# JokerJohn/Cloud_Map_Evaluation

Hardware: AMD Instinct MI355X
Metric: Mpts/sec full metric suite (CD+MME+AWD) on 50M-pt pair (higher is better)
Workload: dtype f64

## Files before the change

cloud_map_evaluation_amd/csrc/me_nn.hip:

```cpp
#include <cmath>
#include <cstdlib>

#include "me_internal.hpp"
#include "me_stat.hpp"

#ifndef ME_NN_DBG
#define ME_NN_DBG 0
#endif

namespace me {

__device__ __forceinline__ double vmin_f64(double a, double b) {
    double r;
    asm("v_min_f64 %0, %1, %2" : "=v"(r) : "v"(a), "v"(b));
    return r;
}

__device__ __forceinline__ float fminf_raw(float a, float b) {
    float r;
    asm("v_min_f32_e32 %0, %1, %2" : "=v"(r) : "v"(a), "v"(b));
    return r;
}

__device__ __forceinline__ double vmax_f64(double a, double b) {
    double r;
    asm("v_max_f64 %0, %1, %2" : "=v"(r) : "v"(a), "v"(b));
    return r;
}

__device__ __forceinline__ double box_lower_bound(const float *__restrict__ b, double qx, double qy, double qz) {
    const double dx = fmax(fmax((double) b[0] - qx, qx - (double) b[3]), 0.0);
    const double dy = fmax(fmax((double) b[1] - qy, qy - (double) b[4]), 0.0);
    const double dz = fmax(fmax((double) b[2] - qz, qz - (double) b[5]), 0.0);
    return (dx * dx + dy * dy) + dz * dz;
}

__device__ __forceinline__ double box_lower_bound_cov(const float *__restrict__ b, double qx, double qy, double qz, int axis, double clo,
                                                      double chi) {
    double d[3];
    d[0] = fmax(fmax((double) b[0] - qx, qx - (double) b[3]), 0.0);
    d[1] = fmax(fmax((double) b[1] - qy, qy - (double) b[4]), 0.0);
    d[2] = fmax(fmax((double) b[2] - qz, qz - (double) b[5]), 0.0);
    const double qa = axis == 0 ? qx : (axis == 1 ? qy : qz);
    const double lo = axis == 0 ? (double) b[0] : (axis == 1 ? (double) b[1] : (double) b[2]);
    const double hi = axis == 0 ? (double) b[3] : (axis == 1 ? (double) b[4] : (double) b[5]);
    if (qa >= clo && qa < chi) {
        const double up = hi >= chi ? fmax(lo, chi) - qa : INFINITY;
        const double dn = lo < clo ? qa - fmin(hi, clo) : INFINITY;
        const double da = fmin(up, dn);
        if (axis == 0) d[0] = da;
        else if (axis == 1) d[1] = da;
        else d[2] = da;
    }
    return (d[0] * d[0] + d[1] * d[1]) + d[2] * d[2];
}

__device__ __forceinline__ double box_upper_bound(const float *__restrict__ b, double qx, double qy, double qz) {
    const double dx = fmax(fabs(qx - (double) b[0]), fabs(qx - (double) b[3]));
    const double dy = fmax(fabs(qy - (double) b[1]), fabs(qy - (double) b[4]));
    const double dz = fmax(fabs(qz - (double) b[2]), fabs(qz - (double) b[5]));
    return (dx * dx + dy * dy) + dz * dz;
}

template <bool FROM_LIST>
__global__ void __launch_bounds__(256) __attribute__((amdgpu_waves_per_eu(8, 8)))
k_nn_grid(const SPoint *__restrict__ qsp, long long q_begin, long long q_end, const SPoint *__restrict__ rsp, long long nr,
          GridView g,
          FrameView fr, SlabView slab, double *__restrict__ d2_out, int *__restrict__ idx_out,
          unsigned int *__restrict__ list, unsigned int *__restrict__ list_count, unsigned int xcd_chunk,
          const unsigned int *__restrict__ in_list, const unsigned int *__restrict__ in_count, unsigned char *__restrict__ flag_out) {
    const int lane = threadIdx.x & 63;
    const unsigned int vb = FROM_LIST ? blockIdx.x : xcd_virtual_block(blockIdx.x, gridDim.x, xcd_chunk);
    const int cell_bits = kMortonBits - g.shift;
    const int cell_lim = 1 << cell_bits;
    const double cell_h = ldexp(fr.fine_h, g.shift);
    __shared__ float4 s_tile[4][64];
    static_assert(sizeof(s_tile[0]) >= kGroupRowsEnt * 4, "the row masks and keys of the round's table alias the wave's tile");
    __shared__ int2 s_tab[4][kGroupTab + 1];
    const unsigned int n_in = FROM_LIST ? *in_count : 0u;
  for (unsigned int pos = vb * blockDim.x + threadIdx.x;; pos += gridDim.x * blockDim.x) {
    unsigned int qoff;
    bool active;
    if (FROM_LIST) {
        if (!__ballot(pos < n_in)) break;
        active = pos < n_in;
        qoff = active ? in_list[pos] : 0u;
    } else {
        qoff = pos;
        active = q_begin + (long long) qoff < q_end;
    }

    double qx = 0, qy = 0, qz = 0;
    int mcx = 0, mcy = 0, mcz = 0;
    bool in_grid = false;
    if (active) {
        unsigned int qo = qoff;
        asm volatile("" : "+v"(qo));
        const SPoint q = qsp[q_begin + (long long) qo];
        qx = q.x;
        qy = q.y;
        qz = q.z;
        if (!FROM_LIST && !slab_owned(slab, qx, qy, qz)) {
            d2_out[q_begin + (long long) qo] = -1.0;
            idx_out[q_begin + (long long) qo] = -1;
            active = false;
        }
    }
    if (active) {
        const double fx = fine_coord(qx, fr.ox, fr.fine_h), fy = fine_coord(qy, fr.oy, fr.fine_h),
                     fz = fine_coord(qz, fr.oz, fr.fine_h);
        const double lim = 2097151.0;
        in_grid = fx >= 0.0 && fy >= 0.0 && fz >= 0.0 && fx <= lim && fy <= lim && fz <= lim;
        if (in_grid) {
            mcx = (int) ((unsigned int) fx >> g.shift);
            mcy = (int) ((unsigned int) fy >> g.shift);
            mcz = (int) ((unsigned int) fz >> g.shift);
        }
    }
    float b1 = INFINITY, b2 = INFINITY, b3 = INFINITY;
    int j1 = -1, j2 = -1;
    bool done = !active || !in_grid;

    float ax = 0, ay = 0, az = 0;
    bool in_round = false;
    const float rank_tol = (float) (1e-3 * cell_h * cell_h);
#if ME_TUNE_NN_SGPR_MASKS
    auto note = [&](float m, int j) {
        unsigned long long lt1, lt2;
        asm("v_cmp_lt_f32_e64 %0, %1, %2" : "=s"(lt1) : "v"(m), "v"(b1));
        asm("v_cmp_lt_f32_e64 %0, %1, %2" : "=s"(lt2) : "v"(m), "v"(b2));
        b3 = __builtin_amdgcn_fmed3f(b2, b3, m);
        b2 = __builtin_amdgcn_fmed3f(b1, b2, m);
        int jn;
        asm("v_cndmask_b32_e64 %0, %1, %2, %3" : "=v"(jn) : "v"(j2), "v"(j), "s"(lt2));
        asm("v_cndmask_b32_e64 %0, %1, %2, %3" : "=v"(j2) : "v"(jn), "v"(j1), "s"(lt1));
        asm("v_min_f32_e32 %0, %1, %2" : "=v"(b1) : "v"(b1), "v"(m));
        asm("v_cndmask_b32_e64 %0, %1, %2, %3" : "=v"(j1) : "v"(j1), "v"(j), "s"(lt1));
    };
#else
    auto note = [&](float m, int j) {
        const bool lt1 = m < b1, lt2 = m < b2;
        b3 = __builtin_amdgcn_fmed3f(b2, b3, m);
        b2 = __builtin_amdgcn_fmed3f(b1, b2, m);
        const int jn = lt2 ? j : j2;
        j2 = lt1 ? j1 : jn;
        b1 = lt1 ? m : b1;
        j1 = lt1 ? j : j1;
    };
#endif
    float4 *tile = s_tile[threadIdx.x >> 6];
    double ox = 0, oy = 0, oz = 0;
    auto rank = [&](int j) {
        const float4 c = tile[j];
        return fmaf(c.x, ax, fmaf(c.y, ay, fmaf(c.z, az, c.w)));
    };
    auto min3 = [](float a, float b, float c) { return __builtin_amdgcn_fmed3f(-INFINITY, a, __builtin_amdgcn_fmed3f(-INFINITY, b, c)); };
    double px64 = 0, py64 = 0, pz64 = 0;
    auto load_chunk = [&](int base, int n) {
        if (lane < n && ME_NN_DBG != 2) {
            const SPoint p = rsp[(ME_NN_DBG == 5) ? ((base + lane) & 4095) : (base + lane)];
            px64 = p.x;
            py64 = p.y;
            pz64 = p.z;
        }
    };
    auto stage_chunk = [&](int n) {
        const int n4 = (n + 3) & ~3;
        if (lane < n4 && ME_NN_DBG != 2) {
            float4 rec = make_float4(0.0f, 0.0f, 0.0f, INFINITY);
            if (lane < n) {
                const double px = px64 - ox, py = py64 - oy, pz = pz64 - oz;
                rec = make_float4((float) px, (float) py, (float) pz, (float) fma(pz, pz, fma(py, py, px * px)));
            }
            tile[lane] = rec;
        }
        __builtin_amdgcn_fence(__ATOMIC_ACQ_REL, "wavefront");
        __builtin_amdgcn_wave_barrier();
    };
    auto rank_chunk = [&](int base, int n) {
        const int n4 = (n + 3) & ~3;
        if (in_round && ME_NN_DBG != 1 && ME_NN_DBG != 2) {
            int j = 0;
#if ME_NN_DBG == 4
            float acc = 0.0f;
            for (; j < n4; ++j) acc += rank(j);
            if (acc == 12345.0f) note(acc, base);
            j = n4;
#endif
            for (; j + 8 <= n4; j += 8) {
                const float m0 = min3(rank(j), rank(j + 1), rank(j + 2));
                const float m1 = min3(rank(j + 3), rank(j + 4), rank(j + 5));
                note(min3(m0, m1, fminf_raw(rank(j + 6), rank(j + 7))), base + j);
            }
            if (j < n4) note(min3(rank(j), rank(j + 1), fminf_raw(rank(j + 2), rank(j + 3))), base + j);
        }
        __builtin_amdgcn_fence(__ATOMIC_ACQ_REL, "wavefront");
        __builtin_amdgcn_wave_barrier();
    };
    int2 *tab = s_tab[threadIdx.x >> 6];
    while (__ballot(!done)) {
        GroupBox bx;
        int nk = 0;
        const bool in = wave_group_table<1, true, kGroupR, false, true>(!done, mcx, mcy, mcz, g, cell_lim, lane, tab, bx, &nk,
                                                  reinterpret_cast<unsigned int *>(tile));
        ox = uniform_f64(fr.ox + (double) bx.x0 * cell_h);
        oy = uniform_f64(fr.oy + (double) bx.y0 * cell_h);
        oz = uniform_f64(fr.oz + (double) bx.z0 * cell_h);
        if (in) {
            unsigned int qo = qoff;
            asm volatile("" : "+v"(qo));
            const SPoint q = qsp[q_begin + (long long) qo];
            ax = (float) (-2.0 * (q.x - ox));
            ay = (float) (-2.0 * (q.y - oy));
            az = (float) (-2.0 * (q.z - oz));
        }
        in_round = in;
        int it_blk = -64, it_pos = 0, it_end = 0;
        unsigned long long it_m = 0;
        auto next_chunk = [&](int &cbase, int &cn) -> bool {
            if (it_pos >= it_end) {
                while (!it_m) {
                    it_blk += 64;
                    if (it_blk >= nk) return false;
                    const int t = it_blk + lane;
                    const int cnt = (t < nk) ? tab[t].y : 0;
                    it_m = __ballot(cnt > 0);
                }
                const int sidx = __ffsll((long long) it_m) - 1;
                it_m &= it_m - 1;
                const int2 run = tab[it_blk + sidx];
                it_pos = __builtin_amdgcn_readfirstlane(run.x);
                it_end = it_pos + __builtin_amdgcn_readfirstlane(run.y);
                while (it_m) {
                    const int s2 = __ffsll((long long) it_m) - 1;
                    const int2 nx = tab[it_blk + s2];
                    if (__builtin_amdgcn_readfirstlane(nx.x) != it_end) break;
                    it_end += __builtin_amdgcn_readfirstlane(nx.y);
                    it_m &= it_m - 1;
                }
            }
            cbase = it_pos;
            cn = min(64, it_end - it_pos);
            it_pos += cn;
            return true;
        };
        int cb = 0, cn = 0;
        bool have = next_chunk(cb, cn);
        if (have) load_chunk(cb, cn);
        while (have) {
            stage_chunk(cn);
            int nb2 = 0, nn2 = 0;
            const bool nhave = next_chunk(nb2, nn2);
            if (nhave) load_chunk(nb2, nn2);
            rank_chunk(cb, cn);
            have = nhave;
            cb = nb2;
            cn = nn2;
        }
        if (in) done = true;
        __builtin_amdgcn_wave_barrier();
    }

    bool unresolved = false;
    if (active) {
        unresolved = true;
        {
            unsigned int qo = qoff;
            asm volatile("" : "+v"(qo));
            const SPoint q = qsp[q_begin + (long long) qo];
            qx = q.x;
            qy = q.y;
            qz = q.z;
        }
        double best_x = INFINITY;
        long long best_i = 0x7fffffffffffffffLL;
        auto exact_group = [&](int jg) {
            if (jg < 0 || ME_NN_DBG == 3) return;
#pragma unroll
            for (int t = 0; t < 8; ++t) {
                const long long pos = (long long) jg + t;
                if (pos < nr) {
                    const SPoint p = rsp[pos];
                    const double e = dist2_exact(qx, qy, qz, p.x, p.y, p.z);
                    if (e < best_x || (e == best_x && p.idx < best_i)) {
                        best_x = e;
                        best_i = p.idx;
                    }
                }
            }
        };
        exact_group(j1);
        if (!(b2 - b1 > rank_tol)) exact_group(j2);
        const bool ranking_safe = b3 - b1 > rank_tol;
        if (in_grid && j1 >= 0 && ranking_safe) {
            const double lox = fr.ox + (double) (mcx - 1) * cell_h, hix = fr.ox + (double) (mcx + 2) * cell_h;
            const double loy = fr.oy + (double) (mcy - 1) * cell_h, hiy = fr.oy + (double) (mcy + 2) * cell_h;
            const double loz = fr.oz + (double) (mcz - 1) * cell_h, hiz = fr.oz + (double) (mcz + 2) * cell_h;
            double gmin = fmin(fmin(qx - lox, hix - qx), fmin(fmin(qy - loy, hiy - qy), fmin(qz - loz, hiz - qz)));
            gmin *= (1.0 - 1e-9);
            unresolved = !(gmin > 0.0 && best_x < gmin * gmin);
        }
        unsigned int qo = qoff;
        asm volatile("" : "+v"(qo));
        d2_out[q_begin + (long long) qo] = best_x;
        idx_out[q_begin + (long long) qo] = (j1 >= 0) ? (int) best_i : -1;
    }
    if (ME_NN_DBG) unresolved = false;
    if (!FROM_LIST && flag_out) {
        if (q_begin + (long long) qoff < q_end) flag_out[qoff] = unresolved ? 1 : 0;
    } else {
        const unsigned long long um = __ballot(unresolved);
        if (um) {
            unsigned int base = 0;
            if (lane == 0) base = atomicAdd(list_count, (unsigned int) __popcll(um));
            base = (unsigned int) readlane_i((int) base, 0);
            if (unresolved) list[base + (unsigned int) __popcll(um & ((1ULL << lane) - 1ULL))] = qoff;
        }
    }
    if (!FROM_LIST) break;
    __builtin_amdgcn_wave_barrier();
  }
}

#ifdef ME_AB
#include "me_nn_kernels_ab.inc"
#endif

__device__ __forceinline__ double octet_min(double v) {
    v = fmin(v, octet_partner_d<0>(v));
    v = fmin(v, octet_partner_d<1>(v));
    v = fmin(v, octet_partner_d<2>(v));
    return v;
}

constexpr int kNn1Block = 64;
constexpr int kNn1Waves = 5;
template <bool COV, bool DBG>
__global__ void __launch_bounds__(kNn1Block) __attribute__((amdgpu_waves_per_eu(kNn1Waves, 8)))
k_nn1(const SPoint *__restrict__ qsp, long long q_begin, long long q_end, const SPoint *__restrict__ rsp, long long nr,
      OctView oct, double *__restrict__ d2_out, int *__restrict__ idx_out, const unsigned int *__restrict__ list,
      const unsigned int *__restrict__ list_count, int use_bound, unsigned long long *__restrict__ dbg,
      unsigned int *__restrict__ far_list, unsigned int *__restrict__ far_count, int far_cap, unsigned int *__restrict__ work,
      const double *__restrict__ cov, int cov_axis) {
    __shared__ long long s_off[kMaxLevels];
    extern __shared__ unsigned int s_dyn[];
    if (threadIdx.x < kMaxLevels) s_off[threadIdx.x] = oct.off[threadIdx.x];
    __syncthreads();
    const int L = oct.n_levels - 1;
    const int lv = oct.n_levels + 1;
    const ONode *__restrict__ nodes = oct.nodes;
    const long long n_items = list ? (long long) *list_count : (q_end - q_begin);
    const int sub = threadIdx.x & 7;
    const unsigned long long t_wave0 = DBG ? wall_clock64() : 0ULL;
    unsigned long long w_open = 0, w_scan = 0, w_pts = 0;
    unsigned int w_max = 0;
    static_assert(kNn1Block == 64, "one wavefront per block: the group counter is drawn by lane 0 of the block");
    for (long long g = blockIdx.x;;) {
        const long long t = g * 8 + (threadIdx.x >> 3);
        const bool alive = t < n_items;
        if (!__ballot(alive)) break;
        {
            unsigned int nx = 0;
            if (threadIdx.x == 0) nx = atomicAdd(work, 1u);
            g = (long long) gridDim.x + (long long) (unsigned int) __builtin_amdgcn_readfirstlane((int) nx);
        }
        const long long i = q_begin + (alive ? (list ? (long long) list[t] : t) : 0);
        const SPoint q = qsp[i];
        const double qx = q.x, qy = q.y, qz = q.z;
        double clo = INFINITY, chi = -INFINITY;
        if (COV && alive) {
            clo = cov[2 * (i - q_begin)];
            chi = cov[2 * (i - q_begin) + 1];
        }
        unsigned int n_open = 0, n_scan = 0;
        unsigned long long n_pts = 0;
        double best = INFINITY;
        long long best_i = 0x7fffffffffffffffLL;
        if (list && alive) {
            best = d2_out[i];
            const int bi = idx_out[i];
            if (bi >= 0) best_i = bi;
        } else if (use_bound && alive) {
            best = d2_out[i];
        }
        double lb = best;
        long long li = best_i;
        double bound = best;
        auto scan_points = [&](bool go, long long jb, long long je) {
            if (!go) jb = je = 0;
            if (DBG) {
                n_scan += go ? 1u : 0u;
                n_pts += (unsigned long long) (je - jb);
            } else {
                n_open += go ? 1u : 0u;
            }
            for (long long j = jb + sub; __ballot(j < je); j += 16) {
                const long long j1 = j + 8;
                const long long last = je > 0 ? je - 1 : 0;
                const SPoint p0 = rsp[j < je ? j : last];
                const SPoint p1 = rsp[j1 < je ? j1 : last];
                const double d0 = dist2_exact(qx, qy, qz, p0.x, p0.y, p0.z);
                const double d1 = dist2_exact(qx, qy, qz, p1.x, p1.y, p1.z);
                if (j < je && (d0 < lb || (d0 == lb && p0.idx < li))) {
                    lb = d0;
                    li = p0.idx;
                }
                if (j1 < je && (d1 < lb || (d1 == lb && p1.idx < li))) {
                    lb = d1;
                    li = p1.idx;
                }
            }
            int m = __float_as_int(__double2float_ru(lb));
            m = min(m, octet_partner_i<0>(m));
            m = min(m, octet_partner_i<1>(m));
            m = min(m, octet_partner_i<2>(m));
            if (go) bound = fmin(bound, (double) __int_as_float(m));
        };
        bool far_flag = false;
        if (L == 0) {
            scan_points(alive, 0, nr);
        } else {
            float *c_lb = reinterpret_cast<float *>(s_dyn) + (threadIdx.x >> 3) * lv * 8;
            unsigned int *c_beg = s_dyn + (kNn1Block / 8) * lv * 8 + (threadIdx.x >> 3) * lv * 9;
            unsigned long long taken_lo = 0, taken_hi = 0;
            bool walking = alive;
            int l = L;
            struct Fetched {
                float4 a, bb;
                unsigned int nxt;
            };
            auto open_load = [&](bool go, int lev, long long cb) {
                if (!go) {
                    cb = 0;
                    lev = 1;
                }
                const long long at = s_off[lev - 1] + cb + sub;
                const float4 *__restrict__ g = reinterpret_cast<const float4 *>(nodes + at);
                Fetched f;
                f.a = g[0];
                f.bb = g[1];
                f.nxt = nodes[at + 1].begin;
                return f;
            };
            auto open_finish = [&](bool go, int lev, long long cb, long long ce, const Fetched &ft) {
                if (!go) {
                    cb = ce = 0;
                    lev = 1;
                }
                const int cnt = (int) (ce - cb);
                n_open += go ? 1u : 0u;
                const float f[6] = {ft.a.x, ft.a.y, ft.a.z, ft.a.w, ft.bb.x, ft.bb.y};
                const bool mine = go && sub < cnt;
                const double ub = octet_min(mine ? box_upper_bound(f, qx, qy, qz) : INFINITY);
                const double lbd = COV ? box_lower_bound_cov(f, qx, qy, qz, cov_axis, clo, chi) : box_lower_bound(f, qx, qy, qz);
                if (go) {
                    bound = fmin(bound, ub);
                    c_lb[lev * 8 + sub] = mine ? __double2float_rd(lbd) : INFINITY;
                    c_beg[lev * 9 + sub] = __float_as_uint(ft.bb.z);
// ... 387 lines not shown
    const long long i = (long long) blockIdx.x * blockDim.x + threadIdx.x;
    bool un = false;
    if (i < n) {
        const double d = d2[i];
        if (d >= 0.0) {
            const SPoint q = qsp[i];
            const double f = slab_face_distance(slab, q.x, q.y, q.z);
            un = !(d < f * f);
        }
    }
    const unsigned long long um = __ballot(un);
    if (um) {
        const int lane = threadIdx.x & 63;
        unsigned int base = 0;
        if (lane == 0) base = atomicAdd(count, (unsigned int) __popcll(um));
        base = (unsigned int) readlane_i((int) base, 0);
        if (un) list[base + (unsigned int) __popcll(um & ((1ULL << lane) - 1ULL))] = (unsigned int) i;
    }
}

__global__ void k_nn_export_xyz(const SPoint *__restrict__ qsp, const unsigned int *__restrict__ list, long long m,
                                double *__restrict__ xyz, const double *__restrict__ d2s, double *__restrict__ d2) {
    const long long t = (long long) blockIdx.x * blockDim.x + threadIdx.x;
    if (t >= m) return;
    const SPoint q = qsp[list[t]];
    if (d2) d2[t] = d2s[list[t]];
    xyz[3 * t] = q.x;
    xyz[3 * t + 1] = q.y;
    xyz[3 * t + 2] = q.z;
}

__global__ void k_points_to_sp(const double *__restrict__ xyz, long long m, SPoint *__restrict__ sp) {
    const long long t = (long long) blockIdx.x * blockDim.x + threadIdx.x;
    if (t >= m) return;
    SPoint p;
    p.x = xyz[3 * t];
    p.y = xyz[3 * t + 1];
    p.z = xyz[3 * t + 2];
    p.idx = t;
    sp[t] = p;
}

__global__ void k_fill_f64(double *p, long long n, double v) {
    const long long t = (long long) blockIdx.x * blockDim.x + threadIdx.x;
    if (t < n) p[t] = v;
}

__global__ void k_nn_patch(const unsigned int *__restrict__ list, long long m, const double *__restrict__ d2_new,
                           double *__restrict__ d2) {
    const long long t = (long long) blockIdx.x * blockDim.x + threadIdx.x;
    if (t >= m) return;
    const unsigned int i = list[t];
    d2[i] = fmin(d2[i], d2_new[t]);
}

static constexpr int nn1_far_cap() { return ME_TUNE_NN1_FAR_CAP <= 0 ? 0x7fffffff : ME_TUNE_NN1_FAR_CAP; }
static constexpr int nn_far_leaf() { return ME_TUNE_NN_FAR_LEAF < 1 ? 1 : ME_TUNE_NN_FAR_LEAF; }
constexpr unsigned int kFarGrid = 1024;
static size_t nn1_cache_bytes(const OctView &oct) { return (size_t) (kNn1Block / 8) * (size_t) (oct.n_levels + 1) * (8 + 9) * 4; }

int nn_search(me_ctx *ctx, int qslot, int rslot) {
    if (qslot < 0 || qslot > 1 || rslot < 0 || rslot > 1) return ctx->fail(ME_ERR_ARG, "bad slot");
    Cloud &q = ctx->cloud[qslot];
    Cloud &r = ctx->cloud[rslot];
    const bool slab = q.slab.axis >= 0;
    if (!q.uploaded || !r.uploaded || (!slab && (!q.index_valid || !r.index_valid)))
        return ctx->fail(ME_ERR_STATE, "me_nn1: upload both clouds first");
    ME_CHECK(ctx, hipSetDevice(ctx->device));
    ME_TRY(cloud_finish_octree(ctx, rslot));
    q.nn_ref_slot = rslot;
    q.surf_have = false;
    q.dfm_have = false;
    ME_TRACE_POINT(ctx, "nn_search: enter");
    q.n_unres = 0;
    if (q.n == 0) return ME_OK;
    ME_CHECK(ctx, q.nn_d2.ensure((size_t) q.n * 8));
    ME_CHECK(ctx, q.nn_idx.ensure((size_t) q.n * 4));
    ME_CHECK(ctx, ctx->red.ensure(64));
    unsigned int *d_cnt = ctx->red.as<unsigned int>();
    long long b, e;
    ctx->shard_range(q.n, b, e);
    if (r.n == 0) {
        hipLaunchKernelGGL(k_nn_fill_empty, dim3((unsigned int) ((q.n + 255) / 256)), dim3(256), 0, ctx->stream, q.sp.as<SPoint>(),
                           q.n, q.slab, q.nn_d2.as<double>(), q.nn_idx.as<int>());
    } else if (e > b) {
        const unsigned int nb = (unsigned int) (((e - b + 255) / 256 + 7) / 8 * 8);
        ME_CHECK(ctx, q.nn_list.ensure((size_t) (e - b) * 4 + 64));
        ME_CHECK(ctx, hipMemsetAsync(d_cnt, 0, 32, ctx->stream));
        FrameView fr{r.origin[0], r.origin[1], r.origin[2], r.fine_h};
        const GridView *levels[Cloud::kMaxMid + 1];
        int n_levels = 0;
        if (r.grid.cell_start && r.grid.shift > r.nn_grid.shift) {
            for (int k = 0; k < r.n_mid; ++k)
                if (r.mid_grid[k].shift > r.nn_grid.shift && r.mid_grid[k].shift < r.grid.shift) levels[n_levels++] = &r.mid_grid[k];
            levels[n_levels++] = &r.grid;
        }
        const bool two_pass = n_levels > 0;
        if (two_pass) {
            ME_CHECK(ctx, ctx->nn_flags.ensure((size_t) (e - b) + 64));
            ME_CHECK(ctx, ctx->nn_list_a.ensure((size_t) (e - b) * 4 + 64));
            if (n_levels > 1) ME_CHECK(ctx, ctx->nn_list_b.ensure((size_t) (e - b) * 4 + 64));
        }
        unsigned int *list_a = two_pass ? ctx->nn_list_a.as<unsigned int>() : q.nn_list.as<unsigned int>();
        unsigned int *cnt_a = two_pass ? d_cnt + 2 : d_cnt;
        {
            TimerScope ts(ctx, "nn_grid");
#ifdef ME_AB
#include "me_nn_dispatch_ab.inc"
#endif
            {
                hipLaunchKernelGGL((k_nn_grid<false>), dim3(nb), dim3(256), 0, ctx->stream, q.sp.as<SPoint>(), b, e, r.sp.as<SPoint>(),
                                   r.n, r.nn_grid, fr, q.slab, q.nn_d2.as<double>(), q.nn_idx.as<int>(), q.nn_list.as<unsigned int>(), d_cnt,
                                   xcd_chunk_setting(), (const unsigned int *) nullptr, (const unsigned int *) nullptr,
                                   two_pass ? ctx->nn_flags.as<unsigned char>() : (unsigned char *) nullptr);
                if (two_pass) ME_TRY(select_flagged_u32(ctx, ctx->nn_flags.as<unsigned char>(), e - b, list_a, cnt_a));
            }
        }
        if (two_pass) {
            TimerScope ts(ctx, "nn_grid2");
            const unsigned int *in_list = list_a, *in_cnt = cnt_a;
            for (int k = 0; k < n_levels; ++k) {
                const bool last = k + 1 == n_levels;
                unsigned int *out_list = last ? q.nn_list.as<unsigned int>() : ((k & 1) ? ctx->nn_list_a.as<unsigned int>() : ctx->nn_list_b.as<unsigned int>());
                unsigned int *out_cnt = last ? d_cnt : ((k & 1) ? d_cnt + 2 : d_cnt + 3);
                if (!last && k >= 1) ME_CHECK(ctx, hipMemsetAsync(out_cnt, 0, 4, ctx->stream));
                hipLaunchKernelGGL((k_nn_grid<true>), dim3(2048), dim3(256), 0, ctx->stream, q.sp.as<SPoint>(), b, e, r.sp.as<SPoint>(), r.n,
                                   *levels[k], fr, q.slab, q.nn_d2.as<double>(), q.nn_idx.as<int>(), out_list, out_cnt, xcd_chunk_setting(),
                                   in_list, in_cnt, (unsigned char *) nullptr);
                in_list = out_list;
                in_cnt = out_cnt;
            }
        }
        {
            const unsigned int nbf = (unsigned int) std::min<long long>((e - b + 7) / 8, 256 * 4 * kNn1Waves);
            ME_CHECK(ctx, ctx->nn_far.ensure((size_t) (e - b) * 4 + 64));
            {
                TimerScope ts(ctx, "nn1");
#define ME_LAUNCH_NN1(COV_, DBG_, DBGP)                                                                                                  \
    hipLaunchKernelGGL((k_nn1<COV_, DBG_>), dim3(nbf), dim3(kNn1Block), nn1_cache_bytes(r.oct), ctx->stream, q.sp.as<SPoint>(), b, e,        \
                       r.sp.as<SPoint>(), r.n, r.oct, q.nn_d2.as<double>(), q.nn_idx.as<int>(), q.nn_list.as<unsigned int>(), d_cnt, 0, DBGP, \
                       ctx->nn_far.as<unsigned int>(), d_cnt + 1, nn1_far_cap(), d_cnt + 4, (const double *) nullptr, 0)
                unsigned long long *dbgp = ctx->timers_on ? ctx->nn1_dbg() : nullptr;
                if (dbgp) ME_LAUNCH_NN1(false, true, dbgp);
                else ME_LAUNCH_NN1(false, false, (unsigned long long *) nullptr);
#undef ME_LAUNCH_NN1
            }
            {
                TimerScope ts(ctx, "nn_far");
                hipLaunchKernelGGL(k_nn_far, dim3(kFarGrid), dim3(256), 0, ctx->stream, q.sp.as<SPoint>(), b, r.sp.as<SPoint>(), r.oct,
                                   q.nn_d2.as<double>(), q.nn_idx.as<int>(), ctx->nn_far.as<unsigned int>(), d_cnt + 1, nn_far_leaf(),
                                   ctx->timers_on ? ctx->nn1_dbg() : nullptr, (const double *) nullptr, 0);
            }
        }
        if (ctx->timers_on) {
            unsigned int h = 0;
            ME_TRY(copy_d2h(ctx, &h, d_cnt, 4));
            ME_CHECK(ctx, hipStreamSynchronize(ctx->stream));
            ctx->nn_fallback += h;
            ctx->nn_queries += e - b;
        }
    }
    if (slab) {
        ME_CHECK(ctx, q.nn_unres.ensure((size_t) q.n * 4 + 64));
        ME_CHECK(ctx, hipMemsetAsync(d_cnt, 0, 4, ctx->stream));
        hipLaunchKernelGGL(k_nn_collect_unresolved, dim3((unsigned int) ((q.n + 255) / 256)), dim3(256), 0, ctx->stream,
                           q.sp.as<SPoint>(), q.n, q.slab, q.nn_d2.as<double>(), q.nn_unres.as<unsigned int>(), d_cnt);
        unsigned int h = 0;
        ME_TRY(copy_d2h(ctx, &h, d_cnt, 4));
        ME_CHECK(ctx, hipStreamSynchronize(ctx->stream));
        q.n_unres = h;
    }
    ME_CHECK(ctx, hipGetLastError());
    return ME_OK;
}

int nn_unresolved(me_ctx *ctx, int qslot, double *xyz_device, double *d2_device, long long capacity, long long *count) {
    if (qslot < 0 || qslot > 1 || !count) return ctx->fail(ME_ERR_ARG, "me_nn_unresolved: bad argument");
    Cloud &q = ctx->cloud[qslot];
    if (q.nn_ref_slot < 0) return ctx->fail(ME_ERR_STATE, "no NN result for this slot (call me_nn1 first)");
    *count = q.n_unres;
    if (!xyz_device || q.n_unres == 0) return ME_OK;
    if (capacity < q.n_unres) return ctx->fail(ME_ERR_CAPACITY, "me_nn_unresolved: capacity too small");
    ME_CHECK(ctx, hipSetDevice(ctx->device));
    hipLaunchKernelGGL(k_nn_export_xyz, dim3((unsigned int) ((q.n_unres + 255) / 256)), dim3(256), 0, ctx->stream, q.sp.as<SPoint>(),
                       q.nn_unres.as<unsigned int>(), q.n_unres, xyz_device, q.nn_d2.as<double>(), d2_device);
    ME_CHECK(ctx, hipStreamSynchronize(ctx->stream));
    return ME_OK;
}

int nn_points(me_ctx *ctx, int rslot, const double *xyz_device, long long m, double *d2_device, bool bounded, int cov_axis,
              const double *cov_device) {
    if (rslot < 0 || rslot > 1 || m < 0 || (m > 0 && (!xyz_device || !d2_device))) return ctx->fail(ME_ERR_ARG, "me_nn_points: bad argument");
    Cloud &r = ctx->cloud[rslot];
    if (!r.uploaded) return ctx->fail(ME_ERR_STATE, "me_nn_points: reference cloud not uploaded");
    if (m == 0) return ME_OK;
    ME_CHECK(ctx, hipSetDevice(ctx->device));
    ME_TRY(cloud_finish_octree(ctx, rslot));
    const unsigned int nb = (unsigned int) ((m + 255) / 256);
    if (r.n == 0) {
        if (!bounded) hipLaunchKernelGGL(k_fill_f64, dim3(nb), dim3(256), 0, ctx->stream, d2_device, m, (double) INFINITY);
    } else {
        DevBuf &qs = ctx->tmp[0], &qi = ctx->tmp[1];
        ME_CHECK(ctx, qs.ensure((size_t) m * sizeof(SPoint)));
        ME_CHECK(ctx, qi.ensure((size_t) m * 4));
        hipLaunchKernelGGL(k_points_to_sp, dim3(nb), dim3(256), 0, ctx->stream, xyz_device, m, qs.as<SPoint>());
        ME_CHECK(ctx, ctx->nn_far.ensure((size_t) m * 4 + 64));
        ME_CHECK(ctx, ctx->red.ensure(64));
        unsigned int *d_cnt = ctx->red.as<unsigned int>();
        ME_CHECK(ctx, hipMemsetAsync(d_cnt, 0, 32, ctx->stream));
        TimerScope ts(ctx, "nn1");
#define ME_LAUNCH_NN1P(COV_, DBG_, DBGP)                                                                                                    \
    hipLaunchKernelGGL((k_nn1<COV_, DBG_>), dim3((unsigned int) std::min<long long>((m + 7) / 8, 256 * 4 * kNn1Waves)), dim3(kNn1Block),        \
                       nn1_cache_bytes(r.oct), ctx->stream, qs.as<SPoint>(), 0LL, m, r.sp.as<SPoint>(), r.n, r.oct, d2_device, qi.as<int>(),    \
                       (const unsigned int *) nullptr, (const unsigned int *) nullptr, bounded ? 1 : 0, DBGP, ctx->nn_far.as<unsigned int>(),   \
                       d_cnt + 1, nn1_far_cap(), d_cnt + 4, cov_device, cov_axis)
        unsigned long long *dbgp = ctx->timers_on ? ctx->nn1_dbg() : nullptr;
        if (cov_device && dbgp) ME_LAUNCH_NN1P(true, true, dbgp);
        else if (cov_device) ME_LAUNCH_NN1P(true, false, (unsigned long long *) nullptr);
        else if (dbgp) ME_LAUNCH_NN1P(false, true, dbgp);
        else ME_LAUNCH_NN1P(false, false, (unsigned long long *) nullptr);
#undef ME_LAUNCH_NN1P
        hipLaunchKernelGGL(k_nn_far, dim3(kFarGrid), dim3(256), 0, ctx->stream, qs.as<SPoint>(), 0LL, r.sp.as<SPoint>(), r.oct, d2_device,
                           qi.as<int>(), ctx->nn_far.as<unsigned int>(), d_cnt + 1, nn_far_leaf(), ctx->timers_on ? ctx->nn1_dbg() : nullptr, cov_device, cov_axis);
    }
    ME_CHECK(ctx, hipStreamSynchronize(ctx->stream));
    ME_CHECK(ctx, hipGetLastError());
    return ME_OK;
}

__global__ void k_cross_message(const SPoint *__restrict__ sp0, const unsigned int *__restrict__ list0, const double *__restrict__ d2s0, long long cnt0,
                                const SPoint *__restrict__ sp1, const unsigned int *__restrict__ list1, const double *__restrict__ d2s1, long long cnt1,
                                long long cap, double n_loc0, double n_loc1, double *__restrict__ msg) {
    const long long t = (long long) blockIdx.x * blockDim.x + threadIdx.x;
    if (t == 0) {
        msg[0] = (double) cnt0;
        msg[1] = (double) cnt1;
        msg[2] = n_loc0;
        msg[3] = n_loc1;
    }
    if (t >= 2 * cap) return;
    const int d = t >= cap ? 1 : 0;
    const long long k = t - d * cap;
    const long long cnt = d ? cnt1 : cnt0;
    double *row = msg + 4 * (1 + t);
    if (k < cnt) {
        const unsigned int at = d ? list1[k] : list0[k];
        const SPoint q = d ? sp1[at] : sp0[at];
        row[0] = q.x;
        row[1] = q.y;
        row[2] = q.z;
        row[3] = d ? d2s1[at] : d2s0[at];
    } else {
        row[0] = row[1] = row[2] = 0.0;
        row[3] = -1.0;
    }
}

struct CrossCuts {
    double c[66];
};
__global__ void k_cross_expand(const double *__restrict__ gathered, int world, long long cap, int dir, int own_rank, CrossCuts cuts, double halo,
                               SPoint *__restrict__ qs, double *__restrict__ bound, double *__restrict__ cov) {
    const long long t = (long long) blockIdx.x * blockDim.x + threadIdx.x;
    if (t >= (long long) world * cap) return;
    const int k = (int) (t / cap);
    const long long j = t - (long long) k * cap;
    const double *row = gathered + 4 * ((long long) k * (1 + 2 * cap) + 1 + (long long) dir * cap + j);
    SPoint p;
    p.x = row[0];
    p.y = row[1];
    p.z = row[2];
    p.idx = t;
    qs[t] = p;
    bound[t] = (k == own_rank) ? -1.0 : row[3];
    cov[2 * t] = cuts.c[k] - halo;
    cov[2 * t + 1] = cuts.c[k + 1] + halo;
}
__global__ void k_cross_collect(const double *__restrict__ gathered, const double *__restrict__ ans, int world, long long cap, int dir, int own_rank,
                                double *__restrict__ d2_out) {
    const long long t = (long long) blockIdx.x * blockDim.x + threadIdx.x;
    if (t >= (long long) world * cap) return;
    const int k = (int) (t / cap);
    const long long j = t - (long long) k * cap;
    const long long at = (long long) k * (1 + 2 * cap) + 1 + (long long) dir * cap + j;
    d2_out[at] = (k == own_rank) ? gathered[4 * at + 3] : ans[t];
    if (j == 0 && dir == 0) d2_out[(long long) k * (1 + 2 * cap)] = 0.0;
}
__global__ void k_cross_untouched(const double *__restrict__ gathered, int world, long long cap, int dir, double *__restrict__ d2_out) {
    const long long t = (long long) blockIdx.x * blockDim.x + threadIdx.x;
    if (t >= (long long) world * cap) return;
    const int k = (int) (t / cap);
    const long long at = (long long) k * (1 + 2 * cap) + 1 + (long long) dir * cap + (t - (long long) k * cap);
    d2_out[at] = gathered[4 * at + 3];
    if (t == (long long) k * cap && dir == 0) d2_out[(long long) k * (1 + 2 * cap)] = 0.0;
}
__global__ void k_cross_patch(const unsigned int *__restrict__ list0, long long cnt0, double *__restrict__ d2_0, const unsigned int *__restrict__ list1,
                              long long cnt1, double *__restrict__ d2_1, const double *__restrict__ mine, long long cap) {
    const long long t = (long long) blockIdx.x * blockDim.x + threadIdx.x;
    if (t < cnt0) {
        const unsigned int i = list0[t];
        d2_0[i] = fmin(d2_0[i], mine[1 + t]);
    } else if (t - cnt0 < cnt1) {
        const long long u = t - cnt0;
        const unsigned int i = list1[u];
        d2_1[i] = fmin(d2_1[i], mine[1 + cap + u]);
    }
// ... 259 lines not shown
```

Measured before the change: 2441.

## Pack candidate runs into dense 64-lane chunks via run list in NN kernel

Replaces the per-run chunk iterator, which issued partial chunks whenever a cell run ended, with a prefix-summed run list (wave_run_list). Each 64-lane load now gathers candidates across run boundaries using a shared-memory head bitmask and mbcnt, so loads and ranking chunks stay full. Ranking pads to groups of 8 instead of 4, and the exact-distance refinement maps a packed position back to a reference index with a binary search over runs. It also adds optional ME_NN_STATS counters. The trade-off is extra LDS atomics, barriers and a binary search per query in exchange for fewer, denser chunks.

```diff
diff --git a/cloud_map_evaluation_amd/csrc/me_nn.hip b/cloud_map_evaluation_amd/csrc/me_nn.hip
--- a/cloud_map_evaluation_amd/csrc/me_nn.hip
+++ b/cloud_map_evaluation_amd/csrc/me_nn.hip
@@ -9,6 +9,10 @@
 #endif
 
 namespace me {
+
+#ifdef ME_NN_STATS
+__device__ unsigned long long g_nn_stat[16];
+#endif
 
 __device__ __forceinline__ double vmin_f64(double a, double b) {
     double r;
@@ -117,95 +121,29 @@
             mcz = (int) ((unsigned int) fz >> g.shift);
         }
     }
-    float b1 = INFINITY, b2 = INFINITY, b3 = INFINITY;
-    int j1 = -1, j2 = -1;
     bool done = !active || !in_grid;
-
-    float ax = 0, ay = 0, az = 0;
-    bool in_round = false;
+    bool unresolved = active;
+    if (active && !in_grid) {
+        unsigned int qo = qoff;
+        asm volatile("" : "+v"(qo));
+        d2_out[q_begin + (long long) qo] = INFINITY;
+        idx_out[q_begin + (long long) qo] = -1;
+    }
+
     const float rank_tol = (float) (1e-3 * cell_h * cell_h);
-#if ME_TUNE_NN_SGPR_MASKS
-    auto note = [&](float m, int j) {
-        unsigned long long lt1, lt2;
-        asm("v_cmp_lt_f32_e64 %0, %1, %2" : "=s"(lt1) : "v"(m), "v"(b1));
-        asm("v_cmp_lt_f32_e64 %0, %1, %2" : "=s"(lt2) : "v"(m), "v"(b2));
-        b3 = __builtin_amdgcn_fmed3f(b2, b3, m);
-        b2 = __builtin_amdgcn_fmed3f(b1, b2, m);
-        int jn;
-        asm("v_cndmask_b32_e64 %0, %1, %2, %3" : "=v"(jn) : "v"(j2), "v"(j), "s"(lt2));
-        asm("v_cndmask_b32_e64 %0, %1, %2, %3" : "=v"(j2) : "v"(jn), "v"(j1), "s"(lt1));
-        asm("v_min_f32_e32 %0, %1, %2" : "=v"(b1) : "v"(b1), "v"(m));
-        asm("v_cndmask_b32_e64 %0, %1, %2, %3" : "=v"(j1) : "v"(j1), "v"(j), "s"(lt1));
-    };
-#else
-    auto note = [&](float m, int j) {
-        const bool lt1 = m < b1, lt2 = m < b2;
-        b3 = __builtin_amdgcn_fmed3f(b2, b3, m);
-        b2 = __builtin_amdgcn_fmed3f(b1, b2, m);
-        const int jn = lt2 ? j : j2;
-        j2 = lt1 ? j1 : jn;
-        b1 = lt1 ? m : b1;
-        j1 = lt1 ? j : j1;
-    };
-#endif
     float4 *tile = s_tile[threadIdx.x >> 6];
-    double ox = 0, oy = 0, oz = 0;
-    auto rank = [&](int j) {
-        const float4 c = tile[j];
-        return fmaf(c.x, ax, fmaf(c.y, ay, fmaf(c.z, az, c.w)));
-    };
-    auto min3 = [](float a, float b, float c) { return __builtin_amdgcn_fmed3f(-INFINITY, a, __builtin_amdgcn_fmed3f(-INFINITY, b, c)); };
-    double px64 = 0, py64 = 0, pz64 = 0;
-    auto load_chunk = [&](int base, int n) {
-        if (lane < n && ME_NN_DBG != 2) {
-            const SPoint p = rsp[(ME_NN_DBG == 5) ? ((base + lane) & 4095) : (base + lane)];
-            px64 = p.x;
-            py64 = p.y;
-            pz64 = p.z;
-        }
-    };
-    auto stage_chunk = [&](int n) {
-        const int n4 = (n + 3) & ~3;
-        if (lane < n4 && ME_NN_DBG != 2) {
-            float4 rec = make_float4(0.0f, 0.0f, 0.0f, INFINITY);
-            if (lane < n) {
-                const double px = px64 - ox, py = py64 - oy, pz = pz64 - oz;
-                rec = make_float4((float) px, (float) py, (float) pz, (float) fma(pz, pz, fma(py, py, px * px)));
-            }
-            tile[lane] = rec;
-        }
-        __builtin_amdgcn_fence(__ATOMIC_ACQ_REL, "wavefront");
-        __builtin_amdgcn_wave_barrier();
-    };
-    auto rank_chunk = [&](int base, int n) {
-        const int n4 = (n + 3) & ~3;
-        if (in_round && ME_NN_DBG != 1 && ME_NN_DBG != 2) {
-            int j = 0;
-#if ME_NN_DBG == 4
-            float acc = 0.0f;
-            for (; j < n4; ++j) acc += rank(j);
-            if (acc == 12345.0f) note(acc, base);
-            j = n4;
-#endif
-            for (; j + 8 <= n4; j += 8) {
-                const float m0 = min3(rank(j), rank(j + 1), rank(j + 2));
-                const float m1 = min3(rank(j + 3), rank(j + 4), rank(j + 5));
-                note(min3(m0, m1, fminf_raw(rank(j + 6), rank(j + 7))), base + j);
-            }
-            if (j < n4) note(min3(rank(j), rank(j + 1), fminf_raw(rank(j + 2), rank(j + 3))), base + j);
-        }
-        __builtin_amdgcn_fence(__ATOMIC_ACQ_REL, "wavefront");
-        __builtin_amdgcn_wave_barrier();
-    };
+    __shared__ unsigned int s_head[4][2];
+    unsigned int *head = s_head[threadIdx.x >> 6];
     int2 *tab = s_tab[threadIdx.x >> 6];
     while (__ballot(!done)) {
         GroupBox bx;
         int nk = 0;
         const bool in = wave_group_table<1, true, kGroupR, false, true>(!done, mcx, mcy, mcz, g, cell_lim, lane, tab, bx, &nk,
                                                   reinterpret_cast<unsigned int *>(tile));
-        ox = uniform_f64(fr.ox + (double) bx.x0 * cell_h);
-        oy = uniform_f64(fr.oy + (double) bx.y0 * cell_h);
-        oz = uniform_f64(fr.oz + (double) bx.z0 * cell_h);
+        const double ox = uniform_f64(fr.ox + (double) bx.x0 * cell_h);
+        const double oy = uniform_f64(fr.oy + (double) bx.y0 * cell_h);
+        const double oz = uniform_f64(fr.oz + (double) bx.z0 * cell_h);
+        float ax = 0, ay = 0, az = 0;
         if (in) {
             unsigned int qo = qoff;
             asm volatile("" : "+v"(qo));
@@ -214,96 +152,186 @@
             ay = (float) (-2.0 * (q.y - oy));
             az = (float) (-2.0 * (q.z - oz));
         }
-        in_round = in;
-        int it_blk = -64, it_pos = 0, it_end = 0;
-        unsigned long long it_m = 0;
-        auto next_chunk = [&](int &cbase, int &cn) -> bool {
-            if (it_pos >= it_end) {
-                while (!it_m) {
-                    it_blk += 64;
-                    if (it_blk >= nk) return false;
-                    const int t = it_blk + lane;
-                    const int cnt = (t < nk) ? tab[t].y : 0;
-                    it_m = __ballot(cnt > 0);
-                }
-                const int sidx = __ffsll((long long) it_m) - 1;
-                it_m &= it_m - 1;
-                const int2 run = tab[it_blk + sidx];
-                it_pos = __builtin_amdgcn_readfirstlane(run.x);
-                it_end = it_pos + __builtin_amdgcn_readfirstlane(run.y);
-                while (it_m) {
-                    const int s2 = __ffsll((long long) it_m) - 1;
-                    const int2 nx = tab[it_blk + s2];
-                    if (__builtin_amdgcn_readfirstlane(nx.x) != it_end) break;
-                    it_end += __builtin_amdgcn_readfirstlane(nx.y);
-                    it_m &= it_m - 1;
-                }
-            }
-            cbase = it_pos;
-            cn = min(64, it_end - it_pos);
-            it_pos += cn;
-            return true;
+        float b1 = INFINITY, b2 = INFINITY, b3 = INFINITY;
+        int j1 = -1, j2 = -1;
+#if ME_TUNE_NN_SGPR_MASKS
+        auto note = [&](float m, int j) {
+            unsigned long long lt1, lt2;
+            asm("v_cmp_lt_f32_e64 %0, %1, %2" : "=s"(lt1) : "v"(m), "v"(b1));
+            asm("v_cmp_lt_f32_e64 %0, %1, %2" : "=s"(lt2) : "v"(m), "v"(b2));
+            b3 = __builtin_amdgcn_fmed3f(b2, b3, m);
+            b2 = __builtin_amdgcn_fmed3f(b1, b2, m);
+            int jn;
+            asm("v_cndmask_b32_e64 %0, %1, %2, %3" : "=v"(jn) : "v"(j2), "v"(j), "s"(lt2));
+            asm("v_cndmask_b32_e64 %0, %1, %2, %3" : "=v"(j2) : "v"(jn), "v"(j1), "s"(lt1));
+            asm("v_min_f32_e32 %0, %1, %2" : "=v"(b1) : "v"(b1), "v"(m));
+            asm("v_cndmask_b32_e64 %0, %1, %2, %3" : "=v"(j1) : "v"(j1), "v"(j), "s"(lt1));
         };
-        int cb = 0, cn = 0;
-        bool have = next_chunk(cb, cn);
-        if (have) load_chunk(cb, cn);
-        while (have) {
-            stage_chunk(cn);
-            int nb2 = 0, nn2 = 0;
-            const bool nhave = next_chunk(nb2, nn2);
-            if (nhave) load_chunk(nb2, nn2);
-            rank_chunk(cb, cn);
-            have = nhave;
-            cb = nb2;
-            cn = nn2;
-        }
-        if (in) done = true;
-        __builtin_amdgcn_wave_barrier();
-    }
-
-    bool unresolved = false;
-    if (active) {
-        unresolved = true;
+#else
+        auto note = [&](float m, int j) {
+            const bool lt1 = m < b1, lt2 = m < b2;
+            b3 = __builtin_amdgcn_fmed3f(b2, b3, m);
+            b2 = __builtin_amdgcn_fmed3f(b1, b2, m);
+            const int jn = lt2 ? j : j2;
+            j2 = lt1 ? j1 : jn;
+            b1 = lt1 ? m : b1;
+            j1 = lt1 ? j : j1;
+        };
+#endif
+        auto rank = [&](int j) {
+            const float4 c = tile[j];
+            return fmaf(c.x, ax, fmaf(c.y, ay, fmaf(c.z, az, c.w)));
+        };
+        auto min3 = [](float a, float b, float c) { return __builtin_amdgcn_fmed3f(-INFINITY, a, __builtin_amdgcn_fmed3f(-INFINITY, b, c)); };
+
+        int n_runs = 0;
+        const int total = wave_run_list(tab, nk, lane, &n_runs);
+        int s_r0 = 0;
+        double px64 = 0, py64 = 0, pz64 = 0;
+        auto load_chunk = [&](int base) {
+            if (ME_NN_DBG == 2) return;
+            if (lane < 2) head[lane] = 0u;
+            __builtin_amdgcn_fence(__ATOMIC_ACQ_REL, "wavefront");
+            __builtin_amdgcn_wave_barrier();
+            if (s_r0 + 1 + lane < n_runs) {
+                const int d = tab[s_r0 + 1 + lane].y - base - 1;
+                if (d < 64) atomicOr(&head[d >> 5], 1u << (d & 31));
+            }
+            __builtin_amdgcn_fence(__ATOMIC_ACQ_REL, "wavefront");
+            __builtin_amdgcn_wave_barrier();
+            const unsigned int h0 = (unsigned int) __builtin_amdgcn_readfirstlane((int) head[0]);
+            const unsigned int h1 = (unsigned int) __builtin_amdgcn_readfirstlane((int) head[1]);
+            if (base + lane < total) {
+                const int2 run = tab[s_r0 + (int) __builtin_amdgcn_mbcnt_hi(h1, __builtin_amdgcn_mbcnt_lo(h0, 0u))];
+                const int gi = run.x + (base + lane - run.y);
+                const SPoint p = rsp[(ME_NN_DBG == 5) ? (gi & 4095) : gi];
+                px64 = p.x;
+                py64 = p.y;
+                pz64 = p.z;
+            }
+            s_r0 += __popc(h0) + __popc(h1);
+        };
+        auto stage_chunk = [&](int n) {
+            const int n8 = (n + 7) & ~7;
+            if (lane < n8 && ME_NN_DBG != 2) {
+                float4 rec = make_float4(0.0f, 0.0f, 0.0f, INFINITY);
+                if (lane < n) {
+                    const double px = px64 - ox, py = py64 - oy, pz = pz64 - oz;
+                    rec = make_float4((float) px, (float) py, (float) pz, (float) fma(pz, pz, fma(py, py, px * px)));
+                }
+                tile[lane] = rec;
+            }
+            __builtin_amdgcn_fence(__ATOMIC_ACQ_REL, "wavefront");
+            __builtin_amdgcn_wave_barrier();
+        };
+        auto rank_chunk = [&](int base, int n) {
+            const int n8 = (n + 7) & ~7;
+            if (in && ME_NN_DBG != 1 && ME_NN_DBG != 2) {
+                int j = 0;
+#if ME_NN_DBG == 4
+                float acc = 0.0f;
+                for (; j < n8; ++j) acc += rank(j);
+                if (acc == 12345.0f) note(acc, base);
+                j = n8;
+#endif
+                for (; j + 8 <= n8; j += 8) {
+                    const float m0 = min3(rank(j), rank(j + 1), rank(j + 2));
+                    const float m1 = min3(rank(j + 3), rank(j + 4), rank(j + 5));
+                    note(min3(m0, m1, fminf_raw(rank(j + 6), rank(j + 7))), base + j);
+                }
+            }
+            __builtin_amdgcn_fence(__ATOMIC_ACQ_REL, "wavefront");
+            __builtin_amdgcn_wave_barrier();
+        };
+#ifdef ME_NN_STATS
+        int st_chunks = 0, st_rec = 0;
+#endif
+        if (total > 0) load_chunk(0);
+        for (int base = 0; base < total; base += 64) {
+            const int n = min(64, total - base);
+            stage_chunk(n);
+            if (base + 64 < total) load_chunk(base + 64);
+            rank_chunk(base, n);
+#ifdef ME_NN_STATS
+            ++st_chunks;
+            st_rec += (n + 7) & ~7;
+#endif
+        }
+#ifdef ME_NN_STATS
         {
+            const int served = __popcll(__ballot(in));
+            if (lane == 0) {
+                unsigned long long *st = g_nn_stat + (FROM_LIST ? 8 : 0);
+                atomicAdd(&st[0], 1ULL);
+                atomicAdd(&st[1], (unsigned long long) st_chunks);
+                atomicAdd(&st[2], (unsigned long long) total);
+                atomicAdd(&st[3], (unsigned long long) st_rec);
+                atomicAdd(&st[4], (unsigned long long) (st_rec >> 3));
+                atomicAdd(&st[6], (unsigned long long) served);
+            }
+        }
+#endif
+        if (in) {
+            double qx, qy, qz;
+            {
+                unsigned int qo = qoff;
+                asm volatile("" : "+v"(qo));
+                const SPoint q = qsp[q_begin + (long long) qo];
+                qx = q.x;
+                qy = q.y;
+                qz = q.z;
+            }
+            double best_x = INFINITY;
+            long long best_i = 0x7fffffffffffffffLL;
+            const int step0 = 1 << (31 - __clz(n_runs | 1));
+            auto exact_group = [&](int jg) {
+                if (jg < 0 || ME_NN_DBG == 3) return;
+                int r = 0;
+                for (int step = step0; step; step >>= 1) {
+                    const int c = r + step;
+                    if (c < n_runs && tab[c].y <= jg) r = c;
+                }
+                int2 cur = tab[r];
+                int nxt = tab[r + 1].y;
+#pragma unroll
+                for (int t = 0; t < 8; ++t) {
+                    const int pos = jg + t;
+                    if (pos < total) {
+                        if (pos >= nxt) {
+                            ++r;
+                            cur = tab[r];
+                            nxt = tab[r + 1].y;
+                        }
+                        const SPoint p = rsp[cur.x + (pos - cur.y)];
+                        const double e = dist2_exact(qx, qy, qz, p.x, p.y, p.z);
+                        if (e < best_x || (e == best_x && p.idx < best_i)) {
+                            best_x = e;
+                            best_i = p.idx;
+                        }
+                    }
+                }
+            };
+            exact_group(j1);
+            if (!(b2 - b1 > rank_tol)) exact_group(j2);
+            const bool ranking_safe = b3 - b1 > rank_tol;
+            if (j1 >= 0 && ranking_safe) {
+                int ux = mcx, uy = mcy, uz = mcz;
+                asm volatile("" : "+v"(ux), "+v"(uy), "+v"(uz));
+                const double lox = fr.ox + (double) (ux - 1) * cell_h, hix = fr.ox + (double) (ux + 2) * cell_h;
+                const double loy = fr.oy + (double) (uy - 1) * cell_h, hiy = fr.oy + (double) (uy + 2) * cell_h;
+                const double loz = fr.oz + (double) (uz - 1) * cell_h, hiz = fr.oz + (double) (uz + 2) * cell_h;
+                double gmin = fmin(fmin(qx - lox, hix - qx), fmin(fmin(qy - loy, hiy - qy), fmin(qz - loz, hiz - qz)));
+                gmin *= (1.0 - 1e-9);
+                unresolved = !(gmin > 0.0 && best_x < gmin * gmin);
+            }
             unsigned int qo = qoff;
             asm volatile("" : "+v"(qo));
-            const SPoint q = qsp[q_begin + (long long) qo];
-            qx = q.x;
-            qy = q.y;
-            qz = q.z;
-        }
-        double best_x = INFINITY;
-        long long best_i = 0x7fffffffffffffffLL;
-        auto exact_group = [&](int jg) {
-            if (jg < 0 || ME_NN_DBG == 3) return;
-#pragma unroll
-            for (int t = 0; t < 8; ++t) {
-                const long long pos = (long long) jg + t;
-                if (pos < nr) {
-                    const SPoint p = rsp[pos];
-                    const double e = dist2_exact(qx, qy, qz, p.x, p.y, p.z);
-                    if (e < best_x || (e == best_x && p.idx < best_i)) {
-                        best_x = e;
-                        best_i = p.idx;
-                    }
-                }
-            }
-        };
-        exact_group(j1);
-        if (!(b2 - b1 > rank_tol)) exact_group(j2);
-        const bool ranking_safe = b3 - b1 > rank_tol;
-        if (in_grid && j1 >= 0 && ranking_safe) {
-            const double lox = fr.ox + (double) (mcx - 1) * cell_h, hix = fr.ox + (double) (mcx + 2) * cell_h;
-            const double loy = fr.oy + (double) (mcy - 1) * cell_h, hiy = fr.oy + (double) (mcy + 2) * cell_h;
-            const double loz = fr.oz + (double) (mcz - 1) * cell_h, hiz = fr.oz + (double) (mcz + 2) * cell_h;
-            double gmin = fmin(fmin(qx - lox, hix - qx), fmin(fmin(qy - loy, hiy - qy), fmin(qz - loz, hiz - qz)));
-            gmin *= (1.0 - 1e-9);
-            unresolved = !(gmin > 0.0 && best_x < gmin * gmin);
-        }
-        unsigned int qo = qoff;
-        asm volatile("" : "+v"(qo));
-        d2_out[q_begin + (long long) qo] = best_x;
-        idx_out[q_begin + (long long) qo] = (j1 >= 0) ? (int) best_i : -1;
+            d2_out[q_begin + (long long) qo] = best_x;
+            idx_out[q_begin + (long long) qo] = (j1 >= 0) ? (int) best_i : -1;
+            done = true;
+        }
+        __builtin_amdgcn_fence(__ATOMIC_ACQ_REL, "wavefront");
+        __builtin_amdgcn_wave_barrier();
     }
     if (ME_NN_DBG) unresolved = false;
     if (!FROM_LIST && flag_out) {
@@ -997,6 +1025,19 @@
                                    ctx->timers_on ? ctx->nn1_dbg() : nullptr, (const double *) nullptr, 0);
             }
         }
+#ifdef ME_NN_STATS
+        {
+            unsigned long long st[16] = {0}, zero[16] = {0};
+            ME_CHECK(ctx, hipStreamSynchronize(ctx->stream));
+            (void) hipMemcpyFromSymbol(st, HIP_SYMBOL(g_nn_stat), sizeof st);
+            (void) hipMemcpyToSymbol(HIP_SYMBOL(g_nn_stat), zero, sizeof zero);
+            for (int k = 0; k < 2; ++k) {
+                const unsigned long long *t = st + 8 * k;
+                if (t[0]) std::fprintf(stderr, "[nn stats] %s queries=%lld rounds=%llu per round: chunks=%.2f lanes/load=%.2f candidates=%.1f ranked records=%.1f note8=%.2f note4=%.2f lanes served=%.1f\n",
+                    k ? "list" : "grid", (long long) (e - b), t[0], (double) t[1] / t[0], (double) t[2] / (double) (t[1] ? t[1] : 1), (double) t[2] / t[0], (double) t[3] / t[0], (double) t[4] / t[0], (double) t[5] / t[0], (double) t[6] / t[0]);
+            }
+        }
+#endif
         if (ctx->timers_on) {
             unsigned int h = 0;
             ME_TRY(copy_d2h(ctx, &h, d_cnt, 4));
```

New measurement: 2517 (median of 6 runs). +3.1%, better.
